# aligokalppeker/hypelcnn

Hardware: AMD Instinct MI355X
Metric: HSI+LiDAR patches/sec fwd+bwd (GRSS2013 7×7×145) at 1/2/4/8 GPU (higher is better)
Workload: dtype f32 (3 x bf16 split operands, 6 partial products, fp32 accumulate); 1 GPU; BASELINE.json configs[1]: GRSS2013 HYPELCNNModel, batch 1024 per GPU, fp32 HIP kernels; train step (fwd+bwd+TF1-Adam), 7x7 patch, 144 HSI + 1 LiDAR bands, 15 classes, alg_param_hypelcnn.json, random-init weights; batch_per_gpu=1024, global_batch=1024, parallelism=single, hip_graph=True

## Files before the change

### hypelcnn_amd/csrc/seg_gemm.hip

```cpp
#include <stdlib.h>

#include <type_traits>
#include <utility>

#include "common.h"

typedef float f32x16 __attribute__((ext_vector_type(16)));
typedef float f32x4 __attribute__((ext_vector_type(4)));
typedef __bf16 bf16x8 __attribute__((ext_vector_type(8)));
typedef __bf16 bf16x2 __attribute__((ext_vector_type(2)));
typedef unsigned u32x2 __attribute__((ext_vector_type(2)));
typedef unsigned u32x4 __attribute__((ext_vector_type(4)));

__device__ __forceinline__ unsigned hypel_cvt_pk_bf16(float a, float b) {
    unsigned r;
    asm("v_cvt_pk_bf16_f32 %0, %1, %2" : "=v"(r) : "v"(a), "v"(b));
    return r;
}
__device__ __forceinline__ void hypel_residual2(float& x0, float& x1, unsigned part) {
    x0 -= __builtin_bit_cast(float, part << 16);
    x1 -= __builtin_bit_cast(float, part & 0xffff0000u);
}
__device__ __forceinline__ void hypel_split2(float x0, float x1, unsigned& h, unsigned& m, unsigned& l) {
    h = hypel_cvt_pk_bf16(x0, x1);
// ... 910 lines not shown
#pragma unroll
                            for (int e = 0; e < 16; ++e) {
                                add[e] = __builtin_bit_cast(float, __builtin_amdgcn_raw_buffer_load_b32(rrs, rvo, so, 0));
                                const int step = (e & 3) == 3 ? 5 * ldr4 : ldr4;
                                asm volatile("s_add_u32 %0, %0, %1" : "+s"(so) : "s"(step) : "scc");
                            }
#pragma unroll
                            for (int e = 0; e < 16; ++e) v[e] += add[e];
                        }
                    }
                    int so = 0;
#pragma unroll
                    for (int e = 0; e < 16; ++e) {
                        __builtin_amdgcn_raw_buffer_store_b32(__builtin_bit_cast(unsigned, v[e]), crs, cvo, so, 0);
                        const int step = (e & 3) == 3 ? 5 * ldc4 : ldc4;
                        asm volatile("s_add_u32 %0, %0, %1" : "+s"(so) : "s"(step) : "scc");
                    }
                } else {
#pragma unroll
                    for (int e = 0; e < 16; ++e)
                        put((wm * TM + i) * 32 + (e & 3) + 8 * (e >> 2) + 4 * lhi, col, acc[i][j][e], bv, o0, o1);
                }
            }
    }
}

#define HYPEL_GEMM_PARAMS                                                                                          \
    const float *__restrict__ A, int64_t lda, const float *__restrict__ B, int64_t ldb, float *__restrict__ C,       \
        int64_t ldc, int n, const hypel_group_t *__restrict__ groups, const hypel_seg_t *__restrict__ segs,           \
        const void *__restrict__ tiles_v, int n_tiles, int n_ntiles, const float *__restrict__ bias, int accumulate, \
        const float *__restrict__ res, int64_t ldr, const int32_t *__restrict__ res_start, float *__restrict__ stats
#define HYPEL_GEMM_ARGS \
    A, lda, B, ldb, C, ldc, n, groups, segs, tiles_v, n_tiles, n_ntiles, bias, accumulate, res, ldr, res_start, stats
#define HYPEL_GEMM_BOUNDS \
    __launch_bounds__(256, (TM * TN == 1 ? (TA ? OCC_BN32_TA : OCC_BN32)                   \
                                         : (TM * TN == 3 ? (TB ? OCC_BN96 : 4) : (TA && TM * TN == 2 ? OCC_BN64_TA : 3))))

template <int WM, int WN, int TM, int TN, bool TA, bool TB, bool NARROW = false, bool MULTI = false, bool PAIR = false,
          bool VARN = false, bool ACT = false>
__global__ HYPEL_GEMM_BOUNDS void seg_gemm_kernel(HYPEL_GEMM_PARAMS) {
    seg_gemm_body<WM, WN, TM, TN, TA, TB, NARROW, MULTI, PAIR, VARN, ACT>(HYPEL_GEMM_ARGS);
}

template <int WM, int WN, int TM, int TN, bool TA, bool TB>
__global__ __attribute__((amdgpu_num_sgpr(96))) HYPEL_GEMM_BOUNDS void seg_gemm_kernel_s96(HYPEL_GEMM_PARAMS) {
    seg_gemm_body<WM, WN, TM, TN, TA, TB>(HYPEL_GEMM_ARGS);
}

template <int WM, int WN, int TM, int TN, bool TA, bool TB, bool MULTI = false>
__global__ __launch_bounds__(64 * WM * WN, (WM * WN == 8 ? 4 : 3)) void seg_gemm_split_kernel(HYPEL_GEMM_PARAMS) {
    seg_gemm_body<WM, WN, TM, TN, TA, TB, false, MULTI, false, false, false, true>(HYPEL_GEMM_ARGS);
}

template <int WM, int WN, int TM, int TN>
int launch_cfg_pair(const float* a, int64_t lda, const float* b, int64_t ldb, float* c, int64_t ldc, int n,
                    const hypel_group_t* groups, const hypel_seg_t* segs, const void* tiles, int n_tiles,
                    const float* bias, int accumulate, const float* res, int64_t ldr, const int32_t* res_start,
                    hipStream_t st) {
    constexpr int BN = WN * TN * 32;
    const int n_nt = (n + BN - 1) / BN;
    hipLaunchKernelGGL((seg_gemm_kernel<WM, WN, TM, TN, false, true, false, false, true>), dim3(n_tiles * n_nt),
                       dim3(256), 0, st, a, lda, b, ldb, c, ldc, n, groups, segs, tiles, n_tiles, n_nt, bias, accumulate,
                       res, ldr, res_start, (float*)nullptr);
    return 0;
}

template <int WM, int WN, int TM, int TN, bool NARROW = false, bool MULTI = false>
int launch_cfg(const float* a, int64_t lda, int ta, const float* b, int64_t ldb, int tb, float* c, int64_t ldc,
               int n, const hypel_group_t* groups, const hypel_seg_t* segs, const void* tiles, int n_tiles,
               const float* bias, int accumulate, const float* res, int64_t ldr, const int32_t* res_start,
               hipStream_t st, float* stats = nullptr, bool cap96 = false) {
    constexpr int BN = NARROW ? 16 * TN : WN * TN * 32;
    const int n_nt = MULTI ? 1 : (n + BN - 1) / BN;
    const int grid = n_tiles * n_nt;
    if constexpr (NARROW && TN > 1) {
        hipLaunchKernelGGL((seg_gemm_kernel<WM, WN, TM, TN, false, false, true, false>), dim3(grid), dim3(256), 0, st, a,
                           lda, b, ldb, c, ldc, n, groups, segs, tiles, n_tiles, n_nt, bias, accumulate, res, ldr,
                           res_start, stats);
        return 0;
    } else {
    if constexpr (TM * TN == 1 && !NARROW && !MULTI) {
        if (cap96 && !ta) {
            if (tb)
                hipLaunchKernelGGL((seg_gemm_kernel_s96<WM, WN, TM, TN, false, true>), dim3(grid), dim3(256), 0, st, a, lda,
                                   b, ldb, c, ldc, n, groups, segs, tiles, n_tiles, n_nt, bias, accumulate, res, ldr,
                                   res_start, stats);
            else
                hipLaunchKernelGGL((seg_gemm_kernel_s96<WM, WN, TM, TN, false, false>), dim3(grid), dim3(256), 0, st, a, lda,
                                   b, ldb, c, ldc, n, groups, segs, tiles, n_tiles, n_nt, bias, accumulate, res, ldr,
                                   res_start, stats);
            return 0;
        }
    }
#define HYPEL_GO(TA_, TB_)                                                                                         \
    hipLaunchKernelGGL((seg_gemm_kernel<WM, WN, TM, TN, TA_, TB_, NARROW, MULTI>), dim3(grid), dim3(256), 0, st, a,  \
                       lda, b, ldb, c, ldc, n, groups, segs, tiles, n_tiles, n_nt, bias, accumulate, res, ldr,     \
                       res_start, stats)
    if constexpr (MULTI) {
        HYPEL_GO(true, false);
    } else {
        if (!ta && !tb) HYPEL_GO(false, false);
        else if (!ta && tb) HYPEL_GO(false, true);
        else HYPEL_GO(true, false);
    }
#undef HYPEL_GO
    return 0;
    }
}

template <int WM, int WN, int TM, int TN, bool MULTI = false>
int launch_split(const float* a, int64_t lda, int ta, const float* b, int64_t ldb, int tb, float* c, int64_t ldc, int n,
                 const hypel_group_t* groups, const hypel_seg_t* segs, const void* tiles, int n_tiles, const float* bias,
                 int accumulate, const float* res, int64_t ldr, const int32_t* res_start, hipStream_t st, float* stats) {
    constexpr int BN = WN * TN * 32;
    const int n_nt = MULTI ? 1 : (n + BN - 1) / BN;
    const int grid = n_tiles * n_nt;
#define HYPEL_GO(TA_, TB_)                                                                                           \
    hipLaunchKernelGGL((seg_gemm_split_kernel<WM, WN, TM, TN, TA_, TB_, MULTI>), dim3(grid), dim3(64 * WM * WN), 0, st, a, lda, b, \
                       ldb, c, ldc, n, groups, segs, tiles, n_tiles, n_nt, bias, accumulate, res, ldr, res_start, stats)
    if constexpr (MULTI) {
        HYPEL_GO(true, false);
    } else {
        if (!ta && !tb) HYPEL_GO(false, false);
        else if (!ta && tb) HYPEL_GO(false, true);
        else HYPEL_GO(true, false);
    }
#undef HYPEL_GO
    return 0;
}

}

static int seg_gemm_dispatch(const float* a, int64_t lda, int32_t trans_a, const float* b, int64_t ldb,
                             int32_t trans_b, float* c, int64_t ldc, int32_t n, const hypel_group_t* groups,
                             const hypel_seg_t* segs, const hypel_tile_t* tiles, int32_t n_tiles, const float* bias,
                             int32_t accumulate, const float* res, int64_t ldr, const int32_t* res_start,
                             hypel_stream_t stream, float* stats = nullptr) {
    HYPEL_REQUIRE(a && b && c && groups && segs && tiles, "hypel_seg_gemm_f32");
    HYPEL_REQUIRE(n > 0 && n_tiles >= 0, "hypel_seg_gemm_f32");
    HYPEL_REQUIRE(!(trans_a && trans_b), "hypel_seg_gemm_f32: A^T B^T products are not part of the path");
    if (n_tiles == 0) return 0;
    hipStream_t st = (hipStream_t)stream;
    int hint = (accumulate >> 8) & 3;
    const bool pairs = (accumulate & HYPEL_GEMM_PAIRED_SEGS) != 0;
    const bool cap96 = (accumulate & HYPEL_GEMM_SINGLE_SEG) != 0;
    const bool mfma16x4 = (accumulate & HYPEL_GEMM_MFMA16X4) != 0;
    const bool var_n = (accumulate & HYPEL_GEMM_VAR_N) != 0;
    const bool split6 = (accumulate & HYPEL_GEMM_SPLIT6) != 0;
    const int act_idx = (accumulate >> 16) & 7;
    accumulate &= 1;
    if (split6) {
        HYPEL_REQUIRE(!pairs && !mfma16x4 && !act_idx && n > 16,
                      "hypel_seg_gemm_f32: HYPEL_GEMM_SPLIT6 needs a plain product with n > 16");
        const int w = hint == 1 || n <= 32 ? 32 : (hint == 2 || n <= 64 ? 64 : (hint == 3 || n > 96 ? 128 : 64));
        (void)var_n;
        if (w == 32)
            launch_split<4, 1, 1, 1>(a, lda, trans_a, b, ldb, trans_b, c, ldc, n, groups, segs, tiles, n_tiles, bias,
                                     accumulate, res, ldr, res_start, st, stats);
        else if (w == 64)
            launch_split<4, 2, 1, 1>(a, lda, trans_a, b, ldb, trans_b, c, ldc, n, groups, segs, tiles, n_tiles, bias,
                                     accumulate, res, ldr, res_start, st, stats);
        else
            launch_split<2, 4, 2, 1>(a, lda, trans_a, b, ldb, trans_b, c, ldc, n, groups, segs, tiles, n_tiles, bias,
                                     accumulate, res, ldr, res_start, st, stats);
        HYPEL_CHECK_LAUNCH("hypel_seg_gemm_f32");
        return 0;
    }
    const bool plain_fwd = !trans_a && !trans_b && !pairs && !stats && !res;
    if (act_idx) {
        HYPEL_REQUIRE(plain_fwd && !accumulate && !mfma16x4 && !var_n && act_idx <= 4,
                      "hypel_seg_gemm_f32: HYPEL_GEMM_ACT_* needs a plain forward product (no accumulate / shortcut / statistics)");
        const bool narrow_a = hint == 1 || n <= 32 || (hint == 0 && (int64_t)n_tiles * ((n + 63) / 64) < 1000);
        const int bn = narrow_a ? 32 : 64;
        const int n_nt = (n + bn - 1) / bn;
        if (narrow_a)
            hipLaunchKernelGGL((seg_gemm_kernel<4, 1, 1, 1, false, false, false, false, false, false, true>),
                               dim3(n_tiles * n_nt), dim3(256), 0, st, a, lda, b, ldb, c, ldc, n, groups, segs, tiles, n_tiles,
                               n_nt, bias, act_idx << 16, res, ldr, res_start, (float*)nullptr);
        else
            hipLaunchKernelGGL((seg_gemm_kernel<4, 1, 1, 2, false, false, false, false, false, false, true>),
                               dim3(n_tiles * n_nt), dim3(256), 0, st, a, lda, b, ldb, c, ldc, n, groups, segs, tiles, n_tiles,
                               n_nt, bias, act_idx << 16, res, ldr, res_start, (float*)nullptr);
        HYPEL_CHECK_LAUNCH("hypel_seg_gemm_f32");
        return 0;
    }
    if (mfma16x4 && n <= 64 && plain_fwd) {
        launch_cfg<4, 1, 1, 4, true>(a, lda, trans_a, b, ldb, trans_b, c, ldc, n, groups, segs, tiles, n_tiles, bias,
                                     accumulate, res, ldr, res_start, st);
        HYPEL_CHECK_LAUNCH("hypel_seg_gemm_f32");
        return 0;
    }
    if (var_n && n > 32 && plain_fwd && hint != 1) {
        const int n_nt = (n + 63) / 64;
        hipLaunchKernelGGL((seg_gemm_kernel<4, 1, 1, 2, false, false, false, false, false, true>),
                           dim3(n_tiles * n_nt), dim3(256), 0, st, a, lda, b, ldb, c, ldc, n, groups, segs, tiles, n_tiles,
                           n_nt, bias, accumulate, res, ldr, res_start, (float*)nullptr);
        HYPEL_CHECK_LAUNCH("hypel_seg_gemm_f32");
        return 0;
    }
    if (hint == 3 && n > 64) {
        launch_cfg<4, 1, 1, 3>(a, lda, trans_a, b, ldb, trans_b, c, ldc, n, groups, segs, tiles, n_tiles, bias,
                               accumulate, res, ldr, res_start, st, stats);
        HYPEL_CHECK_LAUNCH("hypel_seg_gemm_f32");
// ... 92 lines not shown
```

### hypelcnn_amd/plan.py

```python
import os

import numpy as np

from . import graph as G
from .backend import COPY_BLOCK_DTYPE, GEMM_BM, MTILE_DTYPE, REDUCE_ENTRY_DTYPE, SEG_DTYPE, Ref
from .gemm_tables import SEG_PAIR_FLAG, GemmTables, Launch

STAT_CHUNK_ROWS = 256
STAT_BLOCKS = 256


def stat_chunk_rows(rows):
    c = (rows + STAT_BLOCKS - 1) // STAT_BLOCKS
    c = max(16, min(STAT_CHUNK_ROWS, c))
    return (c + 3) // 4 * 4
WGRAD_ROW_CHUNK = 512
TARGET_BLOCKS = 1536
WGRAD_MAX_SPLITS = 64
WGRAD_MIN_SPLITS = 0
DGRAD_MAX_SEGS = 18
MAX_TAPS_PER_TILE = 9
L2_CHUNK_BYTES = int(3.5 * (1 << 20))
SPLITK_BELOW = 400
SPLITK_TARGET = 768
TAP_SPLIT_MIN_BATCH = 64


ACT_IN_GEMM = True
SMALL_BN_ROWS = 1024
MERGE_WGRAD = True


class Storage:

    def __init__(self, buf, nb, ld, pixmap, ch_off, c, npix):
        self.buf = buf
        self.nb = nb
        self.ld = ld
        self.pixmap = pixmap
        self.ch_off = ch_off
        self.c = c
        self.npix = npix

    def pix_off(self, p):
        q = p if self.pixmap is None else self.pixmap[p]
        return q * self.nb * self.ld + self.ch_off

    @property
    def contiguous(self):
        return self.pixmap is None

    @property
    def rows(self):
        return self.npix * self.nb


MSE_PARTIALS = 1024
DP_SYNC_WORK = 0.5
DP_TWO_BUCKET_BYTES = int(float(os.environ.get("HYPEL_DP_TWO_BUCKET_MB", "1048576")) * (1 << 20))
DP_BUCKET_BYTES = int(float(os.environ.get("HYPEL_DP_BUCKET_MB", "256")) * (1 << 20))
DP_MAX_BUCKETS = 8
HINT_OVERRIDE = {k: int(v) for k, v in (kv.split("=") for kv in os.environ.get("HYPEL_HINT_OVERRIDE", "").split(",") if kv)}
RESIDENT_BLOCKS_64 = 6 * 256
GEMM_SINGLE_SEG = 0x800
GEMM_PAIRED_SEGS = 0x400
GEMM_BK = 32
GEMM_SPLIT6 = 0x8000
GEMM_MULTI_SPLIT6 = 0x100
_gs = os.environ.get("HYPEL_GEMM_SPLIT", "6").split(":")
GEMM_SPLIT = int(_gs[0] or 0)
GEMM_SPLIT_WIDTH = int(_gs[1]) if len(_gs) > 1 else 0
GEMM_SPLIT_MIN_FLOPS = float(os.environ.get("HYPEL_GEMM_SPLIT_MIN_GFLOP", "2")) * 1e9
SPLIT_NOMINAL_BATCH = 1024
SPLIT_NOMINAL_BATCH_GAN = 4096
GEMM_SPLIT_MIN_N = 32
SPLIT_OVERRIDE = {k: int(v) for k, v in (kv.split("=") for kv in os.environ.get("HYPEL_SPLIT_OVERRIDE", "").split(",") if kv)}
KSLICE_MIN_GAIN = 0.10
KSLICE_OVERHEAD_K = 24
KSLICE_MIN_K = 48
KSLICE_MAX_SLICES = 16
KSLICE_FRAC_MIN = 0.7
KSLICE_REDUCE_COST_K = 55
KSLICE_SLOTS = {1: 768, 2: 512, 3: 512}
GEMM_MFMA16X4 = 0x2000
GEMM_VAR_N = 0x4000
MERGE_LEVELS = set(x for x in os.environ.get("HYPEL_MERGE_LEVELS", "fwd,dgrad,wgrad").split(",") if x and x != "0")
MERGE_LEVELS_MAX_COUT = 64
MERGE_PASS_MAX_COUT = {"fwd": 16, "dgrad": 1 << 20, "wgrad": 1 << 20}
MERGE_WGRAD_MIN_COUT = 1
MERGE_WGRAD_MAX_COUT = 64
MERGE_FWD_MAX_COUT_SPLIT = 32
MERGE_MAX_TAPS = 0
MERGE_SPLIT_MAX_TAPS = 16
MERGE_SPLIT_KPARTS = False
MERGE_FWD_HINT = 2


for _kv in filter(None, os.environ.get("HYPEL_PLAN_SET", "").split(",")):
    _k, _, _v = _kv.partition("=")
    if not isinstance(globals().get(_k), (bool, int, float)) or _k.startswith("_"):
        raise ValueError(f"HYPEL_PLAN_SET: {_k!r} is not a numeric constant of hypelcnn_amd.plan")
    globals()[_k] = type(globals()[_k])(float(_v)) if not isinstance(globals()[_k], bool) else bool(int(_v))


class TowerPlan:

    _defer_bias_sums = False

    def __init__(self, tower, nb, session, loss=None, labels_c=None, external_masks=False, seed=1234, global_nb=None,
                 sync_bn=False):
        self.tower = tower
        self.nb = int(nb)
        self.global_nb = global_nb
        dist_ = getattr(session, "dist", None)
        self.sync_bn = bool(sync_bn) and dist_ is not None and tower.is_training
        self.world = dist_[0] if dist_ is not None else 1
        self.sess = session
        self.be = session.backend
# ... 112 lines not shown
        order = sorted(groups, key=lambda g: g[0])
        c_min = order[0][0]
        pos = c_min
        for c_off, _, rows in order:
            if c_off != pos:
                return None
            pos += rows * n
        count = pos - c_min
        if c_min % n:
            return None
        a_ks = lda if ta else 1
        b_ks = 1 if tb else ldb
        out = GemmTables()
        for c_off, gs, rows in groups:
            ktot = sum(k for _, _, k in gs)
            cuts = [((ktot * s // S) + 31) // 32 * 32 for s in range(S)] + [ktot]
            cuts = [min(c, ktot) for c in cuts]
            parts = [[] for _ in range(S)]
            base = 0
            for (a_off, b_off, k) in gs:
                for s in range(S):
                    lo, hi = max(cuts[s], base), min(cuts[s + 1], base + k)
                    if hi > lo:
                        parts[s].append((a_off + (lo - base) * a_ks, b_off + (lo - base) * b_ks, hi - lo))
                base += k
            for s in range(S):
                out.add_group(s * count + (c_off - c_min), parts[s], rows)
        return out, S, c_min, count

    @staticmethod
    def _tile_hint(tables, n, ta, tb, folded):
        if n <= 32:
            return 0
        n_tiles = sum((rows + GEMM_BM - 1) // GEMM_BM for _, _, rows in tables.groups)
        blocks64 = n_tiles * ((n + 63) // 64)
        if tb and not ta:
            ks = [k for _, segs, _ in tables.groups for _, _, k in segs]
            if ks and sum(ks) / len(ks) < 48:
                if blocks64 < 1000:
                    return 1
                over = blocks64 % RESIDENT_BLOCKS_64
                return 1 if blocks64 < 2 * RESIDENT_BLOCKS_64 and 0 < over <= RESIDENT_BLOCKS_64 // 10 else 2
            if folded and blocks64 < 4000:
                return 1
            return 1 if blocks64 < 900 else 2
        if ta:
            return 1 if blocks64 < 900 else 2
        if n <= 512 and all(len(segs) == 1 for _, segs, _ in tables.groups):
            if n >= 480 and n % 96 == 0:
                return 3
            return 1
        return 1 if blocks64 < 768 else 2

    def nominal_batch(self):
        return SPLIT_NOMINAL_BATCH

    @staticmethod
    def _split6_width(n):
        if GEMM_SPLIT_WIDTH:
            return GEMM_SPLIT_WIDTH
        if n <= 32:
            return 1
        rem = n % 128
        return 2 if n <= 64 or 0 < rem <= 64 and n < 256 else 3

    def _split6(self, tag, tables, n, ta, tb, flags, paired, in_multi=False):
        eligible = n > 16 and not (ta and tb) and not (flags & ~GEMM_VAR_N) and not paired
        if tag in SPLIT_OVERRIDE:
            w = SPLIT_OVERRIDE[tag]
            if w and not eligible:
                raise ValueError(f"HYPEL_SPLIT_OVERRIDE: launch {tag!r} (n = {n}, trans = {int(bool(ta))}{int(bool(tb))}, "
                                 f"flags = {flags:#x}, paired segments = {bool(paired)}) cannot run on the split-operand "
                                 "kernels (they need n > 16, a plain NN / NT / TN product, no 16x16x4 / activation epilogue)")
            if w not in (0, 1, 2, 3):
                raise ValueError(f"HYPEL_SPLIT_OVERRIDE: width hint {w} for {tag!r} (0 = fp32 kernel, 1 / 2 / 3 = 128x32 / x64 / x128)")
            return w
        if GEMM_SPLIT != 6 or n <= GEMM_SPLIT_MIN_N or not eligible:
            return 0
        if in_multi:
            return self._split6_width(n)
        macs = sum(rows * sum(k for _, _, k in gs) * tables.n_of(gi, n) for gi, (_, gs, rows) in enumerate(tables.groups))
        if 2 * macs * self.nominal_batch() < GEMM_SPLIT_MIN_FLOPS * self.nb:
            return 0
        return self._split6_width(n)

    @staticmethod
    def _kslice_makespan(shares, extra, slots):
        import heapq
        shares = [list(sh) for sh in shares]
        work = [sum(sh) for sh in shares]
        for c in sorted(extra, reverse=True):
            x = min(range(8), key=lambda i: (work[i], i))
            shares[x].append(c)
            work[x] += c
        per = max(1, slots // 8)
        worst = 0.0
        for sh in shares:
            free = [0.0] * per
            for c in sh:
                t = heapq.heappop(free)
                heapq.heappush(free, t + c)
            worst = max(worst, max(free))
        return worst

    def _kslice(self, tables, n, ta, tb, lda, ldb, width_hint):
        groups = tables.groups
# ... 42 lines not shown
                ksum = sum(k for _, _, k in gs)
                s_ = min(KSLICE_MAX_SLICES, -(-ksum // int(T)), max(1, ksum // KSLICE_MIN_K))
                if s_ > 1:
                    sl[gi] = s_
            if sl:
                cands.append(sl)
        per = max(1, slots // 8)
        single_tile_groups = all(rows <= GEMM_BM for _, _, rows in groups)
        for s_ in (2, 3, 4, 6, 8, 12, 16):
            sl = {}
            for share in shares_of(order):
                tail_blocks = (len(share) * ct) % per
                if tail_blocks == 0 or tail_blocks * s_ > per + per // 4:
                    continue
                for t in share[len(share) - (-(-tail_blocks // ct)):]:
                    if t[3] // s_ >= KSLICE_MIN_K:
                        sl[t[2]] = s_
            if sl and single_tile_groups:
                cands.append(sl)
        best, best_t = None, base
        for sl in cands:
            t = evaluate(sl)
            if t < best_t:
                best, best_t = sl, t
        if best is None or best_t > base * (1.0 - KSLICE_MIN_GAIN):
            return None
        return best

    @staticmethod
    def _group_per_tile(tables, lda, ldc):
        out = GemmTables()
        for gi, (c_off, gs, rows) in enumerate(tables.groups):
            for m0 in range(0, rows, GEMM_BM):
                key = tables.keys[gi] if tables.keys[gi] is not None else m0 // GEMM_BM
                out.add_group(c_off + m0 * int(ldc), [(a + m0 * int(lda), b, k) for (a, b, k) in gs], min(GEMM_BM, rows - m0),
                              key=key, subkey=tables.subkeys[gi])
        return out

    @staticmethod
    def _cut_segments(gs, s_, a_ks, b_ks):
        ktot = sum(k for _, _, k in gs)
        cuts = [min(ktot, (ktot * i // s_ + 15) // 16 * 16) for i in range(s_)] + [ktot]
        parts = [[] for _ in range(s_)]
        base = 0
        for (a_off, b_off, k) in gs:
            for i in range(s_):
                lo, hi = max(cuts[i], base), min(cuts[i + 1], base + k)
                if hi > lo:
                    parts[i].append((a_off + (lo - base) * a_ks, b_off + (lo - base) * b_ks, hi - lo))
            base += k
        return parts

    def _emit_gemm(self, lst, tables, n, a_ref, lda, ta, b_ref, ldb, tb, c_ref, ldc, bias_ref, accumulate, tag,
                   allow_split=True, res=None, stats=None, pair=False, hint=None, flags=0, kslice=False, sp6=None):
        split = self._split_k(tables, n, lda, ta, ldb, tb, ldc) if allow_split and res is None else None
        if split is not None:
            stab, S, c_min, count = split
            pos = len(lst)
            self._emit_gemm(lst, stab, n, a_ref, lda, ta, b_ref, ldb, tb, c_ref, ldc, None, 0, tag + "/splitk",
                            allow_split=False)
            self._scratch(lst[pos], 6, "scratch_wgrad", S * count)
            l2 = Launch("reduce_splits_f32", (None, count, S, c_ref + c_min, count, int(accumulate), bias_ref, int(n), 0),
                        nbytes=4 * count * (S + 1), tag="splitk-reduce")
            self._scratch(l2, 0, "scratch_wgrad", S * count)
            lst.append(l2)
            return
        pair = bool(pair and not ta and tb and n > 16 and stats is None)
        if hint is None:
            hint = self._tile_hint(tables, n, ta, tb, res is not None)
        if HINT_OVERRIDE and tag in HINT_OVERRIDE:
            hint = HINT_OVERRIDE[tag]
        single_seg = bool(not ta and all(len(segs) == 1 for _, segs, _ in tables.groups))
        if sp6 is None:
            sp6 = self._split6(tag, tables, n, ta, tb, flags,
                               pair and any(k <= 16 for _, gs, _ in tables.groups for _, _, k in gs))
        if sp6:
            pair, hint, single_seg = False, sp6, False
            accumulate = int(accumulate) | GEMM_SPLIT6
        reduce_after = None
        if (sp6 and kslice and stats is None and not flags and int(ldc) == int(n) and not (ta and tb)
                and tables.groups and not any(tables.ns)):
            per_tile = tables if ta or all(rows <= GEMM_BM for _, _, rows in tables.groups) else self._group_per_tile(tables, lda, ldc)
            slices = self._kslice(per_tile, n, ta, tb, lda, ldb, sp6)
            if slices:
                tables, reduce_after = self._apply_kslices(per_tile, slices, n, lda, ta, ldb, tb, c_ref, ldc, tag)
        garr, sarr, tarr, macs = tables.finalize(n, pair=pair)
        if len(tarr) == 0:
            return
        if pair and tables.paired:
            accumulate = int(accumulate) | GEMM_PAIRED_SEGS
        g_t, s_t, t_t = self.be.upload(garr), self.be.upload(sarr), self.be.upload(tarr)
        self.tables += [g_t, s_t, t_t]
        if single_seg and not flags:
            accumulate = int(accumulate) | GEMM_SINGLE_SEG
        accumulate = int(accumulate) | int(flags)
        args = (a_ref, int(lda), int(ta), b_ref, int(ldb), int(tb), c_ref, int(ldc), int(n), Ref(g_t), Ref(s_t),
                Ref(t_t), int(len(tarr)), bias_ref, int(accumulate) | (hint << 8))
        name = "seg_gemm_f32"
        if res is not None:
            name = "seg_gemm_res_f32"
            args = args + (res[0], int(res[1]), res[2])
        elif stats is not None:
            assert len(tables.groups) == 1 and not (int(accumulate) & 1) and int(ldc) == int(n)
            name = "seg_gemm_stats_f32"
            args = args + (None,)
        l = Launch(name, args, flops=2 * macs, nbytes=tables.compulsory_bytes(n, lda, ta, ldb, tb), tag=tag)
        if stats is not None:
            self._scratch(l, len(args) - 1, "scratch_partial", stats)
        lst.append(l)
        if reduce_after is not None:
            l.meta["kslices"] = reduce_after.meta["kslices"]
            lst.append(reduce_after)

    def _apply_kslices(self, tables, slices, n, lda, ta, ldb, tb, c_ref, ldc, tag):
        from .backend import TILE_PLAIN
        a_ks = int(lda) if ta else 1
        b_ks = 1 if tb else int(ldb)
        kid = self._kslice_bufs
        self._kslice_bufs += 1
        need = sum((s_ - 1) * tables.groups[gi][2] * int(ldc) for gi, s_ in slices.items())
        sname = f"kslice:{kid}"
        self._alloc(sname, need)
        c_rel = self._param_rel(c_ref)
        scratch_from_c = self._param_rel(self._ref(sname)) - c_rel
        out = GemmTables()
        entries, spos = [], 0
        for gi, (c_off, gs, rows) in enumerate(tables.groups):
            s_ = slices.get(gi, 1)
            if s_ == 1:
                out.add_group(c_off, gs, rows, key=tables.keys[gi], subkey=tables.subkeys[gi])
                continue
            parts = self._cut_segments(gs, s_, a_ks, b_ks)
            region = rows * int(ldc)
            out.add_group(c_off, parts[0], rows, key=tables.keys[gi], subkey=tables.subkeys[gi], tail=True)
            for i in range(1, s_):
                out.add_group(scratch_from_c + spos + (i - 1) * region, parts[i], rows, flags=TILE_PLAIN, tail=True)
            entries.append((self._param_rel(self._ref(sname, spos)), c_rel + c_off, region, region, s_ - 1, 1))
            spos += (s_ - 1) * region
        earr = np.array(entries, REDUCE_ENTRY_DTYPE)
        e_t = self.be.upload(earr)
        self.tables.append(e_t)
        red = Launch("reduce_splits_multi_sized_f32", (Ref(self.sess.params), Ref(e_t), int(len(earr)),
                                                       int(max(e[3] for e in entries))),
                     nbytes=4 * sum(cnt * (S + 2) for (_, _, _, cnt, S, _) in entries), tag="kslice-reduce")
        red.meta = {"kslices": {"tiles": len(entries), "slices": int(sum(slices.values())), "of": tag}}
        return out, red

# ... 337 lines not shown
                self.fwd[pos].kparts = kp_used
            for b, col in items:
                self._reduce_tap_copies(ybuf, rows_all, c, col, cout, splits.get(id(b), 1),
                                        None if bias_ref is None else bias_ref + col)

    def _fwd_linear(self, idx, node):
        nb = self.nb
        out = node.out
        c = node.cout
        aux = self._vec_params(node)
        self.node_aux[idx] = aux
        ybuf = f"y:{idx}"
        self._alloc(ybuf, out.npix * nb * c)
        y_st = Storage(ybuf, nb, c, None, 0, c, out.npix)
        aux["y"] = y_st
        bias_ref = self._p(aux["bias"]) if node.has_bias else None

        if node.kind == "conv":
            s_st = self.storage_of(node.sources[0])
            h, w = node.sources[0].hw
            lay = self._level_pass(idx, node, "fwd")
            if lay is not None:
                aux["stats_in_gemm"] = False
                self._fwd_level_merged(node, lay, s_st, ybuf, c, h, w)
            else:
                self._fwd_conv(node, aux, s_st, ybuf, c, h, w, bias_ref)
        elif node.kind == "blockdense":
            src = node.sources[0]
            s_st = self.storage_of(src)
            cout = node.branches[0].cout
            tb = GemmTables()
            for pi, (off, width) in enumerate(node.in_slices):
                tb.add_group(pi * cout, [(s_st.pix_off(0) + off, node.branches[pi].w.offset, width)], nb)
            act_flag = self._act_in_gemm(node, cout)
            aux["act_in_gemm"] = bool(act_flag)
            self._emit_gemm(self.fwd, tb, cout, self._ref(s_st.buf), s_st.ld, 0, Ref(self.sess.params), cout, 0,
                            self._ref(ybuf), c, bias_ref, 0, f"fwd:{node.branches[0].scope}+{len(node.branches) - 1}",
                            allow_split=False, flags=act_flag)
        else:
            b = node.branches[0]
            rowbase = 0
            for si, src in enumerate(node.sources):
                s_st = self.storage_of(src)
                tb = GemmTables()
                segs = [(s_st.pix_off(p), b.w.offset + (rowbase + p * src.c) * c, src.c) for p in range(src.npix)]
                tb.add_group(0, segs, nb)
                act_flag = 0
                if len(node.sources) == 1 and self._split_k(tb, c, s_st.ld, 0, c, 0, c) is None:
                    act_flag = self._act_in_gemm(node, c)
                aux["act_in_gemm"] = bool(act_flag)
                self._emit_gemm(self.fwd, tb, c, self._ref(s_st.buf), s_st.ld, 0, Ref(self.sess.params), c, 0,
                                self._ref(ybuf), c, bias_ref if si == 0 else None, 1 if si > 0 else 0,
                                f"fwd:{b.scope}",
                                flags=act_flag)
                rowbase += src.npix * src.c

        rows = out.npix * nb
        if node.has_bn:
            self._alloc(f"mean:{idx}", c)
            self._alloc(f"rstd:{idx}", c)
            if node.training and self._small_bn(node, rows):
                aux["small_bn"] = True
                aux["mean"] = self._ref(f"mean:{idx}")
            elif node.training and aux.get("stats_in_gemm"):
                n_chunks = (rows + GEMM_BM - 1) // GEMM_BM
                self._emit_bn_finalize(idx, node, aux, n_chunks, GEMM_BM, rows, c)
                aux["mean"] = self._ref(f"mean:{idx}")
            elif node.training:
                chunk = stat_chunk_rows(rows)
                n_chunks = (rows + chunk - 1) // chunk
                l1 = Launch("col_stats_partial", (self._ref(ybuf), c, rows, c, chunk, None),
                            nbytes=4 * rows * c, tag="bn-stats")
                self._scratch(l1, 5, "scratch_partial", n_chunks * 2 * c)
                self.fwd.append(l1)
                self._emit_bn_finalize(idx, node, aux, n_chunks, chunk, rows, c)
                aux["mean"] = self._ref(f"mean:{idx}")
            else:
                self.fwd.append(Launch("rstd_from_var", (self._s(aux["mv"]), c, float(node.bn_eps),
                                                         self._ref(f"rstd:{idx}")), tag="bn-infer"))
                aux["mean"] = self._s(aux["mm"])
            aux["rstd"] = self._ref(f"rstd:{idx}")
            aux["beta_ref"] = self._p(aux["beta"])
        if node.has_post and aux.get("act_in_gemm"):
            self.storage[id(out)] = y_st
        elif node.has_post:
            zbuf = f"z:{idx}"
            self._alloc(zbuf, rows * c)
            self.storage[id(out)] = Storage(zbuf, nb, c, None, 0, c, out.npix)
            self._emit_post_fwd(idx, node, self._ref(ybuf), c, rows, c, aux, self._ref(zbuf))
        else:
            self.storage[id(out)] = y_st

    def _act_in_gemm(self, node, n):
        act = node.act
        if not (ACT_IN_GEMM and node.has_post and not node.has_bn and not node.residuals and node.dropout_keep is None
                and act is not None and act.code == 1 and n > 16 and not self.sync_bn):
            return 0
        for code, slope in ((1, 0.1), (2, 0.18), (3, 0.2), (4, 0.01)):
            if np.float32(act.alpha) == np.float32(slope):
                return code << 16
        return 0

    def _emit_bn_finalize(self, idx, node, aux, n_chunks, chunk, rows, c):
        mean_ref, rstd_ref = self._ref(f"mean:{idx}"), self._ref(f"rstd:{idx}")
        tail = (float(node.bn_eps), mean_ref, rstd_ref, self._s(aux["mm"]), self._s(aux["mv"]), self._bn_decay(node))
        if not self.sync_bn:
            l2 = Launch("bn_finalize", (None, n_chunks, chunk, rows, c) + tail, tag="bn-finalize")
# ... 245 lines not shown
                        copy = h * w * nb * gst.ld
                        for pin, segs in enumerate(per_pixel):
                            for _, si, chunk in self._partial_copies(segs, S):
                                tb.add_group(si * copy + gst.pix_off(pin), chunk, nb, subkey=si)
                        pos = len(self.bwd)
                        self._emit_gemm(self.bwd, tb, src.c, dy, c, 0, w_ref, w_ld or cout, 1,
                                        self._ref(gst.buf), gst.ld, None, 0,
                                        f"dgrad:{items[0][0].scope}/split{mtag}")
                        self._scratch(self.bwd[pos], 6, "scratch_dgrad", S * copy)
                        l2 = Launch("reduce_splits_f32", (None, copy, S, self._ref(gst.buf), h * w * nb * src.c,
                                                          acc, None, src.c, gst.ld),
                                    nbytes=4 * h * w * nb * src.c * (S + 1), tag="dgrad-split-reduce")
                        self._scratch(l2, 0, "scratch_dgrad", S * copy)
                        self.bwd.append(l2)
                        acc = 1
                        continue
                    for pin, segs in enumerate(per_pixel):
                        tb.add_group(gst.pix_off(pin), segs, nb)
                    self._emit_gemm(self.bwd, tb, src.c, dy, c, 0, w_ref, w_ld or cout, 1,
                                    self._ref(gst.buf), gst.ld, None, acc, f"dgrad:{items[0][0].scope}{mtag}",
                                    res=fold_res, pair=cout <= 16, kslice=True)
                    fold_res = None
                    acc = 1
            if trains:
                self._wgrad_conv(idx, node, s_st, dy, c)
        elif node.kind == "blockdense":
            src = node.sources[0]
            s_st = self.storage_of(src)
            cout = node.branches[0].cout
            if self._needs_grad(src):
                gst, acc = self._grad_target(src)
                by_width = {}
                for pi, (off, width) in enumerate(node.in_slices):
                    by_width.setdefault(width, []).append((pi, off))
                for width, items in by_width.items():
                    tb = GemmTables()
                    for pi, off in items:
                        tb.add_group(gst.pix_off(0) + off, [(pi * cout, node.branches[pi].w.offset, cout)], nb)
                    self._emit_gemm(self.bwd, tb, width, dy, c, 0, Ref(self.sess.params), cout, 1, self._ref(gst.buf),
                                    gst.ld, None, acc, f"dgrad:{node.branches[0].scope}+", allow_split=False)
            if trains:
                self._wgrad_blockdense(node, s_st, dy, c, cout)
        else:
            b = node.branches[0]
            rowbase = 0
            for src in node.sources:
                s_st = self.storage_of(src)
                if self._needs_grad(src):
                    gst, acc = self._grad_target(src)
                    tb = GemmTables()
                    for p in range(src.npix):
                        tb.add_group(gst.pix_off(p), [(0, b.w.offset + (rowbase + p * src.c) * c, c)], nb)
                    self._emit_gemm(self.bwd, tb, src.c, dy, c, 0, Ref(self.sess.params), c, 1, self._ref(gst.buf),
                                    gst.ld, None, acc, f"dgrad:{b.scope}")
                rowbase += src.npix * src.c
            if trains:
                self._wgrad_dense(node, dy, c)

    def _emit_post_bwd(self, node, aux, dz, y_ref, rows, c, dy, want_param):
        has_bn = isinstance(node, G.LinearNode) and node.has_bn
        act = node.act
        code, alpha = (act.code, act.alpha) if act else (0, 0.0)
        mean = aux.get("mean") if has_bn else None
        rstd = aux.get("rstd") if has_bn else None
        beta = aux.get("beta_ref") if has_bn else None
        mask = aux.get("mask")
        dparam = None
        if want_param and isinstance(node, G.LinearNode):
            if has_bn:
                dparam = self._g(aux["beta"])
            elif node.has_bias:
                dparam = self._g(aux["bias"])
        if aux.get("small_bn") and has_bn and dy is not None:
            pacc = self._param_acc(aux["beta"]) if dparam is not None else 0
            self.bwd.append(Launch("bn_act_small_bwd", (dz, c, y_ref, c, rows, c, mean, rstd, beta, code, alpha, mask, c,
                                                        dy, c, dparam, pacc), nbytes=16 * rows * c,
                                   tag="post-bwd-small"))
            return
        sums = None
        if has_bn or dparam is not None:
            chunk = stat_chunk_rows(rows)
            n_chunks = (rows + chunk - 1) // chunk
            pacc = 0
            if dparam is not None:
                pacc = self._param_acc(aux["beta"] if has_bn else aux["bias"])
            if not has_bn and dy is not None and (code != 0 or mask is not None) and not self.sync_bn:
                l1 = Launch("act_bias_bwd_reduce", (dz, c, y_ref, c, rows, c, code, alpha, mask, c, chunk, None, dy, c),
                            nbytes=12 * rows * c, tag="post-bwd-reduce+apply")
                if dparam is None:
                    self._scratch(l1, 11, "scratch_partial", n_chunks * 2 * c)
                    self.bwd.append(l1)
                    return
                if self._defer_bias_sums:
                    k = self._bias_sum_bufs
                    self._bias_sum_bufs += 1
                    name = f"bias_sums:{k}"
                    self._alloc(name, n_chunks * 2 * c)
                    args = list(l1.args)
                    args[11] = self._ref(name)
                    l1.args = tuple(args)
                    self.bwd.append(l1)
                    self._bias_sum_entries.append((self._ref(name), dparam, 2 * c, c, n_chunks, pacc))
                    return
                self._scratch(l1, 11, "scratch_partial", n_chunks * 2 * c)
                l2 = Launch("bwd_reduce_finalize", (None, n_chunks, c, None, dparam, pacc), tag="post-bwd-finalize")
                self._scratch(l2, 0, "scratch_partial", n_chunks * 2 * c)
                self._scratch(l2, 3, "sums", 2 * c)
# ... 402 lines not shown
```

### include/hypel.h

```cpp
#ifndef HYPEL_H
#define HYPEL_H
#include <stdint.h>

#ifdef __cplusplus
extern "C" {
#endif

typedef void* hypel_stream_t;

#define HYPEL_ABI_VERSION 8

enum { HYPEL_ACT_NONE = 0, HYPEL_ACT_LRELU = 1, HYPEL_ACT_RELU = 2, HYPEL_ACT_SIGMOID = 3, HYPEL_ACT_TANH = 4 };

int hypel_version(void);
const char* hypel_last_error(void);
int hypel_device_info(int32_t* n_cu, int32_t* n_xcd);

uint32_t hypel_crc32c(uint32_t crc, const void* data, uint64_t n);

int hypel_nhwc_to_pnc(const float* x, float* out, int64_t n, int32_t p, int32_t c, int64_t ld,
                      hypel_stream_t stream);
int hypel_pnc_to_nhwc(const float* in, int64_t ld, float* x, int64_t n, int32_t p, int32_t c,
                      hypel_stream_t stream);
int hypel_fill_f32(float* dst, int64_t count, float value, hypel_stream_t stream);

typedef struct { int64_t a_off; int64_t b_off; int32_t k; int32_t reserved; } hypel_seg_t;
typedef struct { int64_t c_off; int32_t seg_begin; int32_t seg_count; int32_t rows; int32_t reserved; } hypel_group_t;
typedef struct {
    int32_t group; int32_t m0;
    int32_t rows; int32_t seg_begin; int32_t seg_count;
    int32_t k0; int64_t c_off; int64_t a_off0; int64_t b_off0;
    int32_t flags; int32_t n;
} hypel_tile_t;
#define HYPEL_GEMM_BM 128
#define HYPEL_TILE_PLAIN 1
#define HYPEL_SEG_PAIR_FLAG 0x40000000
#define HYPEL_GEMM_PAIRED_SEGS 0x400
#define HYPEL_GEMM_SINGLE_SEG 0x800

#define HYPEL_GEMM_MFMA16X4 0x2000
#define HYPEL_GEMM_VAR_N 0x4000
#define HYPEL_GEMM_ACT_LRELU_0_1 0x10000
#define HYPEL_GEMM_ACT_LRELU_0_18 0x20000
#define HYPEL_GEMM_ACT_LRELU_0_2 0x30000
#define HYPEL_GEMM_ACT_LRELU_0_01 0x40000
#define HYPEL_GEMM_SPLIT6 0x8000
#define HYPEL_GEMM_MULTI_SPLIT6 0x100

int hypel_seg_gemm_f32(const float* a, int64_t lda, int32_t trans_a, const float* b, int64_t ldb, int32_t trans_b,
                       float* c, int64_t ldc, int32_t n, const hypel_group_t* groups, const hypel_seg_t* segs,
                       const hypel_tile_t* tiles, int32_t n_tiles, const float* bias, int32_t accumulate,
                       hypel_stream_t stream);

int hypel_seg_gemm_stats_f32(const float* a, int64_t lda, int32_t trans_a, const float* b, int64_t ldb,
                             int32_t trans_b, float* c, int64_t ldc, int32_t n, const hypel_group_t* groups,
                             const hypel_seg_t* segs, const hypel_tile_t* tiles, int32_t n_tiles, const float* bias,
                             int32_t accumulate, float* stats_partial, hypel_stream_t stream);

int hypel_seg_gemm_res_f32(const float* a, int64_t lda, int32_t trans_a, const float* b, int64_t ldb, int32_t trans_b,
                           float* c, int64_t ldc, int32_t n, const hypel_group_t* groups, const hypel_seg_t* segs,
                           const hypel_tile_t* tiles, int32_t n_tiles, const float* bias, int32_t accumulate,
                           const float* res, int64_t ldr, const int32_t* res_start, hypel_stream_t stream);

typedef struct {
    int64_t c_off; int64_t a_off0; int64_t b_off0;
    int32_t m0; int32_t rows; int32_t n0; int32_t n;
    int32_t seg_begin; int32_t seg_count; int32_t k0; int32_t flags;
    int32_t lda; int32_t ldb; int32_t ldc; int32_t reserved;
} hypel_mtile_t;
int hypel_seg_gemm_multi_f32(const float* base, int32_t trans_a, int32_t trans_b, int32_t tile_width,
                             const hypel_seg_t* segs, const hypel_mtile_t* blocks, int32_t n_blocks,
                             hypel_stream_t stream);

typedef struct {
    int64_t partial_off; int64_t out_off; int64_t stride; int64_t count; int32_t n_splits; int32_t flags;
} hypel_reduce_entry_t;
int hypel_reduce_splits_multi_f32(const float* base, const hypel_reduce_entry_t* entries, int32_t n_entries,
                                  hypel_stream_t stream);
int hypel_reduce_splits_multi_sized_f32(const float* base, const hypel_reduce_entry_t* entries, int32_t n_entries,
                                        int64_t max_count, hypel_stream_t stream);

int hypel_reduce_splits_wave_multi_f32(const float* base, const hypel_reduce_entry_t* entries, int32_t n_entries,
                                       int64_t total_count, hypel_stream_t stream);

int hypel_reduce_splits_f32(const float* partial, int64_t stride, int32_t n_splits, float* out, int64_t count,
                            int32_t accumulate, const float* bias, int32_t n, int64_t ldc, hypel_stream_t stream);

int hypel_reduce_splits_pair_f32(const float* partial0, int64_t stride0, int64_t count0, float* out0,
                                 const float* partial1, int64_t stride1, int64_t count1, float* out1, int32_t n_splits,
                                 int32_t accumulate, hypel_stream_t stream);

// ... 342 lines not shown
```

Before: 181,900 patches/s.

## Add split-K short GEMM kernel for small-N dense layers

Adds a new GEMM kernel for dense (1-pixel) layers with a single segment, moderate K and small N. Each of the four waves handles a slice of K using native fp32 MFMA 16x16x4 with buffer loads, and the partial sums are reduced through shared memory. The planner flags qualifying forward and dgrad dense GEMMs so they use this path. The goal is to raise block count and parallelism for skinny GEMMs that the tiled kernel underfills. In exchange it bypasses the bf16 split path and adds a shared-memory reduction.

```diff
diff --git a/hypelcnn_amd/csrc/seg_gemm.hip b/hypelcnn_amd/csrc/seg_gemm.hip
--- a/hypelcnn_amd/csrc/seg_gemm.hip
+++ b/hypelcnn_amd/csrc/seg_gemm.hip
@@ -986,6 +986,153 @@
     seg_gemm_body<WM, WN, TM, TN, TA, TB, false, MULTI, false, false, false, true>(HYPEL_GEMM_ARGS);
 }
 
+template <int RT, bool TB>
+__global__ __launch_bounds__(256) void seg_gemm_short_kernel(const float* __restrict__ A, int64_t lda,
+                                                             const float* __restrict__ B, int64_t ldb,
+                                                             float* __restrict__ C, int64_t ldc, int n,
+                                                             const hypel_tile_t* __restrict__ tiles, int n_tiles,
+                                                             int n_ntiles, const float* __restrict__ bias,
+                                                             int accumulate) {
+    constexpr int BM = 16 * RT, BN = 32, SUB = HYPEL_GEMM_BM / BM, NACC = 2 * RT;
+    constexpr int U = RT == 4 ? 4 : 8;
+    constexpr int PLANE = NACC * 256;
+    __shared__ float part[4 * PLANE];
+
+    const int nblk = gridDim.x;
+    const int bid = blockIdx.x;
+    const int xcd = bid & 7, loc = bid >> 3;
+    const int qb = nblk >> 3, rb = nblk & 7;
+    const int lid = (xcd < rb ? xcd * (qb + 1) : rb * (qb + 1) + (xcd - rb) * qb) + loc;
+    const int per_tile = n_ntiles * SUB;
+    const int tile_id = lid / per_tile;
+    if (tile_id >= n_tiles) return;
+    const int rem = lid - tile_id * per_tile;
+    const int sub = rem / n_ntiles;
+    const int n0 = (rem - sub * n_ntiles) * BN;
+    const hypel_tile_t t = tiles[tile_id];
+    if (t.n > 0) n = t.n;
+    if (t.flags & HYPEL_TILE_PLAIN) {
+        bias = nullptr;
+        accumulate = 0;
+    }
+    const int m0 = t.m0 + sub * BM;
+    const int rows_left = t.rows - m0;
+    const int cols_left = n - n0;
+    if (rows_left <= 0 || cols_left <= 0) return;
+    const int K = t.seg_count > 0 ? t.k0 : 0;
+
+    const int tid = threadIdx.x;
+    const int lane = tid & 63;
+    const int wave = __builtin_amdgcn_readfirstlane(tid >> 6);
+    const int r = lane & 15, q = lane >> 4;
+    const int ls = ((K + 15) >> 4) << 2;
+    const int ks = wave * ls;
+    const int len = __builtin_amdgcn_readfirstlane(max(0, min(K - ks, ls)));
+    const int steps = (len + 3) >> 2;
+    const int rows_valid = min(BM, rows_left), cols_valid = min(BN, cols_left);
+    const int kOOB = 0x7fffffff;
+    const int lda4 = __builtin_amdgcn_readfirstlane((int)lda * 4), ldb4 = __builtin_amdgcn_readfirstlane((int)ldb * 4);
+
+    const float* const pa = A + t.a_off0 + (int64_t)m0 * lda + ks;
+    const float* const pb = TB ? B + t.b_off0 + (int64_t)n0 * ldb + ks : B + t.b_off0 + (int64_t)ks * ldb + n0;
+    int voff_a[RT], voff_b[2];
+#pragma unroll
+    for (int i = 0; i < RT; ++i) voff_a[i] = 16 * i + r < rows_valid ? (16 * i + r) * lda4 + 4 * q : kOOB;
+#pragma unroll
+    for (int c = 0; c < 2; ++c)
+        voff_b[c] = 16 * c + r < cols_valid ? (TB ? (16 * c + r) * ldb4 + 4 * q : q * ldb4 + 4 * (16 * c + r)) : kOOB;
+
+    auto load = [&](auto& ra, auto& rbv, int j0) {
+        const int kb = 4 * j0;
+        const int left = __builtin_amdgcn_readfirstlane(min(len - kb, 4 * U));
+        const int span_a = left > 0 ? (rows_valid - 1) * lda4 + 4 * left : 0;
+        const int span_b = left > 0 ? (TB ? (cols_valid - 1) * ldb4 + 4 * left : (left - 1) * ldb4 + 4 * cols_valid) : 0;
+        const __amdgpu_buffer_rsrc_t rsa = __builtin_amdgcn_make_buffer_rsrc(
+            (void*)(pa + kb), 0, __builtin_amdgcn_readfirstlane(span_a), 0x00020000);
+        const __amdgpu_buffer_rsrc_t rsb = __builtin_amdgcn_make_buffer_rsrc(
+            (void*)(TB ? pb + kb : pb + (int64_t)kb * ldb), 0, __builtin_amdgcn_readfirstlane(span_b), 0x00020000);
+#pragma unroll
+        for (int u = 0; u < U; ++u) {
+            const bool k_ok = 4 * u + q < left;
+#pragma unroll
+            for (int i = 0; i < RT; ++i)
+                ra[u][i] = __builtin_bit_cast(float, __builtin_amdgcn_raw_buffer_load_b32(
+                                                         rsa, k_ok && voff_a[i] != kOOB ? voff_a[i] + 16 * u : kOOB, 0, 0));
+#pragma unroll
+            for (int c = 0; c < 2; ++c)
+                rbv[u][c] = __builtin_bit_cast(
+                    float, __builtin_amdgcn_raw_buffer_load_b32(
+                               rsb, k_ok && voff_b[c] != kOOB ? voff_b[c] + (TB ? 16 * u : 4 * u * ldb4) : kOOB, 0, 0));
+        }
+    };
+
+    f32x4 acc[RT][2];
+#pragma unroll
+    for (int i = 0; i < RT; ++i)
+#pragma unroll
+        for (int c = 0; c < 2; ++c)
+#pragma unroll
+            for (int e = 0; e < 4; ++e) acc[i][c][e] = 0.0f;
+    auto mma = [&](const auto& ra, const auto& rbv) {
+#pragma unroll
+        for (int u = 0; u < U; ++u)
+#pragma unroll
+            for (int i = 0; i < RT; ++i)
+#pragma unroll
+                for (int c = 0; c < 2; ++c)
+                    acc[i][c] = __builtin_amdgcn_mfma_f32_16x16x4f32(ra[u][i], rbv[u][c], acc[i][c], 0, 0, 0);
+    };
+
+    float a0[U][RT], b0[U][2], a1[U][RT], b1[U][2];
+    load(a0, b0, 0);
+    for (int j0 = 0; j0 < steps; j0 += 2 * U) {
+        load(a1, b1, j0 + U);
+        mma(a0, b0);
+        load(a0, b0, j0 + 2 * U);
+        if (j0 + U < steps) mma(a1, b1);
+    }
+
+    float* const pw = part + wave * PLANE;
+#pragma unroll
+    for (int i = 0; i < RT; ++i)
+#pragma unroll
+        for (int c = 0; c < 2; ++c)
+#pragma unroll
+            for (int e = 0; e < 4; ++e) pw[((i * 2 + c) * 4 + e) * 64 + lane] = acc[i][c][e];
+    __syncthreads();
+
+    float* const cbase = C + t.c_off + (int64_t)m0 * ldc + n0;
+    const int bias_col0 = bias ? (int)(t.c_off % ldc) + n0 : 0;
+    const int col = tid & 31;
+    const float bv = bias && col < cols_left ? bias[bias_col0 + col] : 0.0f;
+#pragma unroll
+    for (int p = 0; p < 2 * RT; ++p) {
+        const int row = (tid >> 5) + 8 * p;
+        const int rr = row & 15;
+        const int off = (((row >> 4) * 2 + (col >> 4)) * 4 + (rr & 3)) * 64 + (col & 15) + 16 * (rr >> 2);
+        float v = ((part[off] + part[off + PLANE]) + part[off + 2 * PLANE]) + part[off + 3 * PLANE];
+        if (row < rows_left && col < cols_left) {
+            float* const dst = cbase + (int64_t)row * ldc + col;
+            v += bv;
+            if (accumulate) v += *dst;
+            *dst = v;
+        }
+    }
+}
+
+template <int RT>
+void launch_short(const float* a, int64_t lda, const float* b, int64_t ldb, int tb, float* c, int64_t ldc, int n,
+                  const hypel_tile_t* tiles, int n_tiles, const float* bias, int accumulate, hipStream_t st) {
+    const int n_nt = (n + 31) / 32;
+    const int grid = n_tiles * n_nt * (HYPEL_GEMM_BM / (16 * RT));
+    if (tb)
+        hipLaunchKernelGGL((seg_gemm_short_kernel<RT, true>), dim3(grid), dim3(256), 0, st, a, lda, b, ldb, c, ldc, n,
+                           tiles, n_tiles, n_nt, bias, accumulate);
+    else
+        hipLaunchKernelGGL((seg_gemm_short_kernel<RT, false>), dim3(grid), dim3(256), 0, st, a, lda, b, ldb, c, ldc, n,
+                           tiles, n_tiles, n_nt, bias, accumulate);
+}
+
 template <int WM, int WN, int TM, int TN>
 int launch_cfg_pair(const float* a, int64_t lda, const float* b, int64_t ldb, float* c, int64_t ldc, int n,
                     const hypel_group_t* groups, const hypel_seg_t* segs, const void* tiles, int n_tiles,
@@ -1082,7 +1229,19 @@
     const bool var_n = (accumulate & HYPEL_GEMM_VAR_N) != 0;
     const bool split6 = (accumulate & HYPEL_GEMM_SPLIT6) != 0;
     const int act_idx = (accumulate >> 16) & 7;
+    const bool shortm = (accumulate & HYPEL_GEMM_SHORT) != 0;
     accumulate &= 1;
+    if (shortm && cap96 && !trans_a && !res && !stats && !pairs && !mfma16x4 && !var_n && !act_idx && !split6) {
+        const int n_nt = (n + 31) / 32;
+        if (n_nt >= 16)
+            launch_short<4>(a, lda, b, ldb, trans_b, c, ldc, n, tiles, n_tiles, bias, accumulate, st);
+        else if (n_nt >= 8)
+            launch_short<2>(a, lda, b, ldb, trans_b, c, ldc, n, tiles, n_tiles, bias, accumulate, st);
+        else
+            launch_short<1>(a, lda, b, ldb, trans_b, c, ldc, n, tiles, n_tiles, bias, accumulate, st);
+        HYPEL_CHECK_LAUNCH("hypel_seg_gemm_f32");
+        return 0;
+    }
     if (split6) {
         HYPEL_REQUIRE(!pairs && !mfma16x4 && !act_idx && n > 16,
                       "hypel_seg_gemm_f32: HYPEL_GEMM_SPLIT6 needs a plain product with n > 16");
diff --git a/hypelcnn_amd/plan.py b/hypelcnn_amd/plan.py
--- a/hypelcnn_amd/plan.py
+++ b/hypelcnn_amd/plan.py
@@ -64,6 +64,10 @@
 RESIDENT_BLOCKS_64 = 6 * 256
 GEMM_SINGLE_SEG = 0x800
 GEMM_PAIRED_SEGS = 0x400
+GEMM_SHORT = 0x1000
+GEMM_SHORT_MAX_KN = 1 << 19
+GEMM_SHORT_MIN_K = 96
+GEMM_SHORT_MAX_N = 160
 GEMM_BK = 32
 GEMM_SPLIT6 = 0x8000
 GEMM_MULTI_SPLIT6 = 0x100
@@ -282,6 +286,16 @@
             return 1
         return 1 if blocks64 < 768 else 2
 
+    @staticmethod
+    def _short_layer(tables, n):
+        if GEMM_SHORT_MAX_KN <= 0 or len(tables.groups) != 1 or any(tables.ns):
+            return False
+        _, segs, _ = tables.groups[0]
+        if len(segs) != 1:
+            return False
+        k = segs[0][2]
+        return k >= GEMM_SHORT_MIN_K and int(n) <= GEMM_SHORT_MAX_N and k * int(n) <= GEMM_SHORT_MAX_KN
+
     def nominal_batch(self):
         return SPLIT_NOMINAL_BATCH
 
@@ -430,8 +444,12 @@
         return parts
 
     def _emit_gemm(self, lst, tables, n, a_ref, lda, ta, b_ref, ldb, tb, c_ref, ldc, bias_ref, accumulate, tag,
-                   allow_split=True, res=None, stats=None, pair=False, hint=None, flags=0, kslice=False, sp6=None):
+                   allow_split=True, res=None, stats=None, pair=False, hint=None, flags=0, kslice=False, sp6=None,
+                   dense=False):
         split = self._split_k(tables, n, lda, ta, ldb, tb, ldc) if allow_split and res is None else None
+        short = bool(dense and split is None and res is None and stats is None and not pair and not flags and not ta
+                     and self._short_layer(tables, n)
+                     and not (self._split6(tag, tables, n, ta, tb, flags, False) if sp6 is None else sp6))
         if split is not None:
             stab, S, c_min, count = split
             pos = len(lst)
@@ -471,6 +489,8 @@
         self.tables += [g_t, s_t, t_t]
         if single_seg and not flags:
             accumulate = int(accumulate) | GEMM_SINGLE_SEG
+        if short:
+            accumulate = int(accumulate) | GEMM_SHORT
         accumulate = int(accumulate) | int(flags)
         args = (a_ref, int(lda), int(ta), b_ref, int(ldb), int(tb), c_ref, int(ldc), int(n), Ref(g_t), Ref(s_t),
                 Ref(t_t), int(len(tarr)), bias_ref, int(accumulate) | (hint << 8))
@@ -914,7 +934,7 @@
                 self._emit_gemm(self.fwd, tb, c, self._ref(s_st.buf), s_st.ld, 0, Ref(self.sess.params), c, 0,
                                 self._ref(ybuf), c, bias_ref if si == 0 else None, 1 if si > 0 else 0,
                                 f"fwd:{b.scope}",
-                                flags=act_flag)
+                                flags=act_flag, dense=out.npix == 1)
                 rowbase += src.npix * src.c
 
         rows = out.npix * nb
@@ -1266,7 +1286,7 @@
                     for p in range(src.npix):
                         tb.add_group(gst.pix_off(p), [(0, b.w.offset + (rowbase + p * src.c) * c, c)], nb)
                     self._emit_gemm(self.bwd, tb, src.c, dy, c, 0, Ref(self.sess.params), c, 1, self._ref(gst.buf),
-                                    gst.ld, None, acc, f"dgrad:{b.scope}")
+                                    gst.ld, None, acc, f"dgrad:{b.scope}", dense=node.out.npix == 1)
                 rowbase += src.npix * src.c
             if trains:
                 self._wgrad_dense(node, dy, c)
diff --git a/include/hypel.h b/include/hypel.h
--- a/include/hypel.h
+++ b/include/hypel.h
@@ -37,6 +37,7 @@
 #define HYPEL_SEG_PAIR_FLAG 0x40000000
 #define HYPEL_GEMM_PAIRED_SEGS 0x400
 #define HYPEL_GEMM_SINGLE_SEG 0x800
+#define HYPEL_GEMM_SHORT 0x1000
 
 #define HYPEL_GEMM_MFMA16X4 0x2000
 #define HYPEL_GEMM_VAR_N 0x4000
```

Result: no change. 182,300 patches/s (median of 6 runs) (+0.3%).
